# meteorologytoday/XLab-FFTBarotropic

Measured on AMD Instinct MI355X. Metric: RK4 steps/sec, 4096x4096 periodic grid, higher is better.
Workload: dtype f32; 1 GPU; 4096x4096 kuo2004 initial field, nu=6.5, L=600 km, dt=0.75 s, 4 RK stages/step, fused HIP path; parallelism=single

## Files before the change

### xlab-fftbarotropic_amd/csrc/fb_col_full.h

```cpp
#pragma once
#include "fb_kernels.h"

#define CF_THREADS 1024
#define CF_X1_CF 16384
#define CF_X2_STR 68
#define CF_X2_CF (16 * 16 * CF_X2_STR)
#define CF_GX_CF 2048
#define CF_LDS_CF (CF_X2_CF + 512 + CF_GX_CF)
#define CF_LDS_BYTES (CF_LDS_CF * 8)
#ifndef CF_KEEP1
#define CF_KEEP1 5
#endif
#ifndef CF_KEEP2
#define CF_KEEP2 5
#endif

struct FullArgs {
    const cf *Tin;
    const cf *Zbase;
    cf *Zcur, *Acc, *Zout;
    cf *W4;
    long fstride;
    int P;
    int ntiles;
    int ntiles_run;
    int nsub;
    int stage;
    float nu, dt;
    SpecCoef coef;
    const cf *tw256;
    const cf *tw4096;
    long sub_rows;
    float wscale;
};

FB_DEV void cf_xchg_waves(cf *lds, cf *v, int w, int lane)
{
#pragma unroll
    for (int r = 0; r < 16; ++r) lds_wr(&lds[(r * 16 + w) * 64 + lane], v[r]);
    lds_barrier();
#pragma unroll
    for (int r = 0; r < 16; ++r) v[r] = lds_rd(&lds[(w * 16 + r) * 64 + lane]);
    lds_barrier();
}

template <bool SYNC>
FB_DEV void cf_xchg_lanes(cf *lds, cf *v, int w, int l, int c)
{
    cf *reg = lds + w * (16 * CF_X2_STR);
#pragma unroll
    for (int r = 0; r < 16; ++r) lds_wr(&reg[r * CF_X2_STR + l * 4 + c], v[r]);
    __builtin_amdgcn_wave_barrier();
#pragma unroll
    for (int r = 0; r < 16; ++r) v[r] = lds_rd(&reg[l * CF_X2_STR + r * 4 + c]);
    if (SYNC) lds_barrier();
    else { asm volatile("s_waitcnt lgkmcnt(0)" ::: "memory"); __builtin_amdgcn_wave_barrier(); }
}

#define CF_FENCE() __builtin_amdgcn_sched_barrier(0)
FB_DEV cf cf_mul(cf a, cf b) { return cmul_split(a, b); }
FB_DEV cf cf_mulc(cf a, cf b) { return cmulc_split(a, b); }

template <int DIR> FB_DEV void cf_bfly16(cf *v)
{
    fft4<DIR>(v[0], v[4], v[8], v[12]);  CF_FENCE();
    fft4<DIR>(v[1], v[5], v[9], v[13]);  CF_FENCE();
// ... 191 lines not shown
#pragma unroll
        for (int k3 = 0; k3 < KEEP; ++k3) zkeep[k3] = cf_ld4(ZN + k3 * sstep, voff_s);
    }
#pragma unroll 1
    for (int f = 0; f < 4; ++f) {
        if (f > 0 || PRIME) {
            const unsigned vs = (unsigned)launder((int)voff_s);
#pragma unroll
            for (int k3 = 0; k3 < 16; ++k3) {
                const float4 z = k3 < KEEP ? zkeep[k3] : cf_ld4(ZN + k3 * sstep, vs);
                v[0][k3] = cf_make(z.x, z.y); v[1][k3] = cf_make(z.z, z.w);
            }
        }
        const bool psi = f >= 2, use_gx = (f == 0 || f == 3);
        const int lkx = launder(l);
#pragma unroll
        for (int k3 = 0; k3 < 16; ++k3) {
            cf za = v[0][k3], zb = v[1][k3];
            const float gx = gxt[16 * w + 256 * k3 + lkx];
            if (psi) {
                const double kx2 = (double)gx * (double)gx;
                const float lia = (nsub * (w + 256 * k3 + 16 * l) + k1 == 0 && ky0 == 0) ? 1.0f : (float)(-(kx2 + ky2_of(gya)));
                const float lib = (float)(-(kx2 + ky2_of(gyb)));
                za = pada ? cf_make(0.f, 0.f) : cf_make(za.x / lia, za.y / lia);
                zb = padb ? cf_make(0.f, 0.f) : cf_make(zb.x / lib, zb.y / lib);
            }
            const float ka = (use_gx ? gx : gya) * a.wscale, kb = (use_gx ? gx : gyb) * a.wscale;
            v[0][k3] = cf_make(-za.y * ka, za.x * ka);
            v[1][k3] = cf_make(-zb.y * kb, zb.x * kb);
            CF_FENCE();
        }
        cf_fft4096<+1, (KEEP > 0)>(lds, tabA, tabB, v, w, KEEP > 0 ? lkx : l, c, lane);
        char *dst = reinterpret_cast<char *>(a.W4) + (size_t)f * a.fstride * sizeof(cf) + ubase_m;
        const unsigned vm = (unsigned)launder((int)voff_m);
#pragma unroll
        for (int i = 0; i < 16; ++i)
            cf_st4_w4(dst + i * rstep, vm, make_float4(v[0][i].x, v[0][i].y, v[1][i].x, v[1][i].y));
    }
}

template <bool TO_FULL>
__global__ void __launch_bounds__(256) k_full_relayout(const cf *__restrict__ in, cf *__restrict__ out, int P, int N1, int N2, int ntiles, int nsub, int hy)
{
    const size_t total = (size_t)nsub * (ntiles + 1) * 16 * CF_THREADS * 2;
    for (size_t idx = (size_t)blockIdx.x * blockDim.x + threadIdx.x; idx < total; idx += (size_t)gridDim.x * blockDim.x) {
        const int col = (int)(idx & 1);
        const int tid = (int)((idx >> 1) & (CF_THREADS - 1));
        const int k3 = (int)((idx >> 11) & 15);
        const int st = (int)(idx >> 15);
        const int k1 = st / (ntiles + 1), tile = st - k1 * (ntiles + 1);
        const int w = tid >> 6, l = (tid >> 2) & 15, c = tid & 3;
        const int kx = nsub * (w + 16 * l + 256 * k3) + k1, ky = tile * 8 + 2 * c + col;
        const int cc = kx % N1, d = kx / N1;
        const size_t p3 = (size_t)(N2 * cc + d) * P + ky;
        if (ky >= hy) { if (TO_FULL) out[idx] = cf_make(0.f, 0.f); continue; }
        if (TO_FULL) out[idx] = in[p3]; else out[p3] = in[idx];
    }
}
```

### xlab-fftbarotropic_amd/csrc/fb_rowq.h

```cpp
#pragma once
#include "fb_rowh.h"

#define RQ_LAUNDER(t) (SLAB ? launder(t) : (t))
struct RowQ {
    static constexpr int M = 2048, N = 4096, T = 256;
    static constexpr int SLICE = Row8::SLICE;
    static constexpr int XBUF = 4 * SLICE;
    static constexpr int STG = M + 2;
    static constexpr int TW2 = 64;
    static constexpr size_t LDS_BYTES = (size_t)(XBUF + STG + TW2) * sizeof(cf);
};
struct RowQTw { cf w0[7], w1[3]; const cf *w2; };

FB_DEV void rq_xch_group_bwd(cf *v, cf *xbuf, int w, int l)
{
#pragma unroll
    for (int p = 0; p < 8; ++p) lds_wr(&xbuf[(p & 3) * RowQ::SLICE + ((p >> 2) * 4 + w) * 64 + l], v[p]);
    lds_barrier();
#pragma unroll
    for (int j = 0; j < 8; ++j) v[j] = lds_rd(&xbuf[w * RowQ::SLICE + j * 64 + l]);
}
FB_DEV void rq_xch_group_fwd(cf *v, cf *xbuf, int w, int l)
{
#pragma unroll
// ... 18 lines not shown
#pragma unroll
        for (int q = 1; q < 4; ++q) v[4 * h + q] = cmulc(v[4 * h + q], tw.w1[q - 1]);
    }
    r8_xch_wave<true>(v, slice, l_hi, l_lo);
    Bfly<8, +1>::run(v);
#pragma unroll
    for (int p = 1; p < 8; ++p) v[p] = cmulc(v[p], lds_rd(&tw.w2[p * 8 + l_lo]));
    r8_xch_wave<false>(v, slice, l_hi, l_lo);
    Bfly<8, +1>::run(v);
}

FB_DEV void rq_fwd(cf *v, cf *xbuf, const RowQTw &tw, int w, int l)
{
    const int l_hi = l >> 3, l_lo = l & 7;
    cf *slice = xbuf + w * RowQ::SLICE;
    Bfly<8, -1>::run(v);
    r8_xch_wave<false>(v, slice, l_hi, l_lo);
#pragma unroll
    for (int p = 1; p < 8; ++p) v[p] = cmul(v[p], lds_rd(&tw.w2[p * 8 + l_lo]));
    Bfly<8, -1>::run(v);
    r8_xch_wave<true>(v, slice, l_hi, l_lo);
#pragma unroll
    for (int h = 0; h < 2; ++h) {
#pragma unroll
        for (int q = 1; q < 4; ++q) v[4 * h + q] = cmul(v[4 * h + q], tw.w1[q - 1]);
        fft4<-1>(v[4 * h], v[4 * h + 1], v[4 * h + 2], v[4 * h + 3]);
    }
    rq_xch_group_fwd(v, xbuf, w, l);
#pragma unroll
    for (int p = 1; p < 8; ++p) v[p] = cmul(v[p], tw.w0[p - 1]);
    Bfly<8, -1>::run(v);
}

template <bool SLAB>
FB_DEV void rq_dma_issue(cf *stg, int t, const RowView &view, int field, int row)
{
    constexpr int M = RowQ::M;
    const int w = t >> 6, lane = t & 63;
#pragma unroll
    for (int c = 0; c < 4; ++c) {
        const int ch = w + c * 4, k = ch * 128 + lane * 2;
        __builtin_amdgcn_global_load_lds((const void __attribute__((address_space(1))) *)row_ptr<SLAB>(view, field, row, k), rh_to_lds(stg + ch * 128), 16, 0, 2);
    }
    rh_lds_ptr nyq = rh_to_lds(stg + M);
    const float *src = reinterpret_cast<const float *>(row_ptr<SLAB>(view, field, row, M)) + (t & 1);
    if (t < 2) __builtin_amdgcn_global_load_lds((const void __attribute__((address_space(1))) *)src, nyq, 4, 0, 0);
}

FB_DEV void rq_ext(cf *v, int t, const cf *stg, const cf *wk)
{
    constexpr int M = RowQ::M;
#pragma unroll
    for (int e = 0; e < 8; ++e) {
        const int k = t + 256 * e;
        cf a = lds_rd(&stg[k]), b = lds_rd(&stg[M - k]);
        if (e == 0 && t == 0) { a.y = 0.f; b.y = 0.f; }
        const cf ev = cadd_conj(a, b);
        cf d = cmul(csub_conj(a, b), wk[e == 4 ? 0 : e]);
        if (e == 4) d = mul_w16<4, +1>(d);
        v[e] = cadd_ib(ev, d);
    }
}

FB_DEV int rq_phys(int t, int e)
{
    const int w = t >> 6, l = t & 63, l_hi = l >> 3, l_lo = l & 7;
    return (w + 4 * (l_hi >> 2)) + 8 * (l_hi & 3) + 32 * l_lo + 256 * e;
}

__global__ void __launch_bounds__(256) k_rowq_permute_src(const float *__restrict__ in, float *__restrict__ out, int nrows)
{
    constexpr int M = RowQ::M;
    const size_t total = (size_t)nrows * M;
    for (size_t idx = (size_t)blockIdx.x * blockDim.x + threadIdx.x; idx < total; idx += (size_t)gridDim.x * blockDim.x) {
        const int x = (int)(idx / M), r = (int)(idx - (size_t)x * M);
        const int t = r & 255, e = r >> 8;
        reinterpret_cast<float2 *>(out)[idx] = reinterpret_cast<const float2 *>(in)[(size_t)x * M + rq_phys(t, e)];
    }
}

template <bool SLAB, bool PRE = false>
__global__ void __launch_bounds__(256, 4) k_rowq(RowArgs a, const float4 *__restrict__ tab )
{
    constexpr int M = RowQ::M;
    extern __shared__ __attribute__((aligned(16))) unsigned char smem_raw[];
    cf *xbuf = reinterpret_cast<cf *>(smem_raw);
    cf *stg = xbuf + RowQ::XBUF;
    const int t = threadIdx.x, l = t & 63;
    const bool valid = (int)blockIdx.x < a.nx;
    const int x = a.x0 + (valid ? (int)blockIdx.x : 0);
    rq_dma_issue<SLAB>(stg, t, a.M, 0, x);
    RowQTw tw;
    cf wkn[8];
    cf *tw2 = stg + RowQ::STG;
    {
        float4 q[9];
#pragma unroll
        for (int j = 0; j < 9; ++j) q[j] = tab[j * 256 + t];
        tw.w0[0] = cf_make(q[0].x, q[0].y); tw.w0[1] = cf_make(q[0].z, q[0].w); tw.w0[2] = cf_make(q[1].x, q[1].y); tw.w0[3] = cf_make(q[1].z, q[1].w);
        tw.w0[4] = cf_make(q[2].x, q[2].y); tw.w0[5] = cf_make(q[2].z, q[2].w); tw.w0[6] = cf_make(q[3].x, q[3].y);
        tw.w1[0] = cf_make(q[3].z, q[3].w); tw.w1[1] = cf_make(q[4].x, q[4].y); tw.w1[2] = cf_make(q[4].z, q[4].w);
        wkn[0] = cf_make(q[5].x, -q[5].y);
        if (t < 64) tw2[t] = cf_make(q[5].z, q[5].w);
        wkn[1] = cf_make(q[6].x, -q[6].y); wkn[2] = cf_make(q[6].z, -q[6].w); wkn[3] = cf_make(q[7].x, -q[7].y);
        wkn[5] = cf_make(q[7].z, -q[7].w); wkn[6] = cf_make(q[8].x, -q[8].y); wkn[7] = cf_make(q[8].z, -q[8].w);
        wkn[4] = wkn[0];
    }
    tw.w2 = tw2;
#pragma unroll
    for (int p = 0; p < 7; ++p) asm volatile("" :: "v"(tw.w0[p]));
    asm volatile("" :: "v"(tw.w1[0]), "v"(tw.w1[1]), "v"(tw.w1[2]), "v"(wkn[0]), "v"(wkn[7]));
    RH_WAIT_ROW();
    __syncthreads();

    for (int once = 0; once < 1; ++once) {
        cf v[8], p[8];
        auto c2r_phase = [&](bool wait, int next_field, int next_row) {
            const int tp = RQ_LAUNDER(t);
            if (wait) RH_WAIT_ROW();
            lds_barrier();
            rq_ext(v, tp, stg, wkn);
            lds_barrier();
            if (next_row >= 0) rq_dma_issue<SLAB>(stg, tp, a.M, next_field, next_row);
            rq_bwd(v, xbuf, tw, tp >> 6, tp & 63);
        };
        c2r_phase(false, 2, x);
#pragma unroll
        for (int e = 0; e < 8; ++e) p[e] = PRE ? v[e] : cf_make(v[e].x * a.scale, v[e].y * a.scale);
        c2r_phase(true, 1, x);
#pragma unroll
        for (int e = 0; e < 8; ++e) p[e] = PRE ? cf_make(v[e].x * p[e].x, v[e].y * p[e].y) : cf_make((v[e].x * a.scale) * p[e].x, (v[e].y * a.scale) * p[e].y);
        c2r_phase(true, 3, x);
        {
            cf zy[8];
#pragma unroll
            for (int e = 0; e < 8; ++e) zy[e] = PRE ? v[e] : cf_make(v[e].x * a.scale, v[e].y * a.scale);
            c2r_phase(true, 0, -1);
#pragma unroll
            for (int e = 0; e < 8; ++e)
                v[e] = PRE ? cf_make(p[e].x - v[e].x * zy[e].x, p[e].y - v[e].y * zy[e].y)
                           : cf_make(p[e].x - (v[e].x * a.scale) * zy[e].x, p[e].y - (v[e].y * a.scale) * zy[e].y);
        }
        const int tt = RQ_LAUNDER(t);
        if (a.src && a.src_nz[x]) {
            const float2 *sp = reinterpret_cast<const float2 *>(a.src) + (size_t)x * M + tt;
#pragma unroll
            for (int e = 0; e < 8; ++e) { const float2 q = sp[e * 256]; v[e].x += q.x; v[e].y += q.y; }
        }
        rq_fwd(v, xbuf, tw, tt >> 6, tt & 63);
        RH_WAIT_ROW();
        lds_barrier();
#pragma unroll
        for (int e = 4; e < 8; ++e) lds_wr(&xbuf[tt + 256 * (e - 4)], v[e]);
        lds_barrier();
        if (valid) {
#pragma unroll
// ... 24 lines not shown
```

### xlab-fftbarotropic_amd/csrc/fftbaro.hip

```cpp
#include <hip/hip_runtime.h>
#include <algorithm>
#include <cmath>
#include <cstdio>
#include <cstdlib>
#include <cstring>
#include <mutex>
#include <set>
#include <string>
#include <type_traits>
#include <utility>
#include <vector>

#include "../../include/fftbaro.h"
#include "fb_kernels.h"
#include "fb_keff.h"
#include "fb_azim.h"
#include "fb_census.h"
#include "fb_spectra.h"
#include "fb_tracer.h"
#include "fb_particles.h"
#include "fb_tangent.h"
#include "fb_clv.h"
#include "fb_adjoint.h"
#include "fb_obs.h"
// ... 54 lines not shown
    RK_GENERIC,
    RK_ROWQ,
    RK_ROW8,
    RK_ROWH_8192,
    RK_ROWH_16384,
    RK_ROWH2,
};
enum XPass {
    XP_COLS = 0,
    XP_FULL1 = 1,
    XP_FULL2 = 2,
};

struct fb_ctx {
    int world, rank;
    int XL;
    int ngroups, nact; ColGroup grp[3];
    int KA, KF, katot;
    int nx, ny, hy, P;
    int N1, N2;
    int jmax;
    float lx, ly;
    hipStream_t stream;
    RowKernel row;
    float *d_gx; double *d_kx2; float *d_gy; double *d_ky2; double gws;
    cf *d_tw_n1, *d_tw_n2, *d_tw_big, *d_tw_row_bwd, *d_tw_row_fwd, *d_tw_256;
    cf *d_tw_row3;
    cf *d_tw_4096;
    cf *d_tw_2048;
    bool rowq_off, no_row8, no_rowh;
    bool full_pass_off, full_noskip;
    bool no_column_skip, no_prescale;
    bool full_keep_off;
    int pitch_extra;
    bool no_pitch_tune, pitch_tune, tune_verbose;
    bool nyq_frozen;
    cf *d_scratch;
    std::vector<float> h_gx, h_gy; std::vector<double> h_kx2, h_ky2;
    int max_wg;
    int dev;
};

static void split_nx(int nx, int &N1, int &N2)
{
    if (nx % 3 == 0) { N1 = 24; N2 = nx / 24; return; }
    switch (nx) {
    case 64: N1 = 8; N2 = 8; break;
    case 128: N1 = 16; N2 = 8; break;
    case 256: N1 = 16; N2 = 16; break;
    case 512: N1 = 32; N2 = 16; break;
    case 1024: N1 = 32; N2 = 32; break;
    case 2048: N1 = 64; N2 = 32; break;
    case 4096: N1 = 64; N2 = 64; break;
    case 8192: N1 = 128; N2 = 64; break;
    default: N1 = 128; N2 = 128; break;
    }
}

static std::vector<cf> make_root_table(int n)
{
    std::vector<cf> t(n);
    for (int j = 0; j < n; ++j) {
        double a = -2.0 * M_PI * (double)j / (double)n;
        t[j].x = (float)cos(a); t[j].y = (float)sin(a);
    }
    return t;
// ... 45 lines not shown
    for (int s = 0; s < RowPlan<N>::S; ++s) r.push_back(RowTw<N, false>::radix(s));
    if (fwd) r = std::vector<int>(r.rbegin(), r.rend());
    return r;
}

static std::vector<int> plan_radices_rt(int n, bool fwd)
{
    switch (n) {
    case 64: return plan_radices<64>(fwd);
    case 128: return plan_radices<128>(fwd);
    case 256: return plan_radices<256>(fwd);
    case 512: return plan_radices<512>(fwd);
    case 1024: return plan_radices<1024>(fwd);
    case 2048: return plan_radices<2048>(fwd);
    case 4096: return plan_radices<4096>(fwd);
    case 8192: return plan_radices<8192>(fwd);
    default: return plan_radices<16384>(fwd);
    }
}

template <typename T> static int upload(T **dptr, const std::vector<T> &h)
{
    HIPCHK(hipMalloc((void **)dptr, h.size() * sizeof(T)));
    HIPCHK(hipMemcpy(*dptr, h.data(), h.size() * sizeof(T), hipMemcpyHostToDevice));
    return FB_OK;
}

static int autotune_pitch(fb_ctx *c);

static void read_switches(fb_ctx *c)
{
    auto set = [](const char *name) { return getenv(name) != nullptr; };
    const char *rowq = getenv("FB_ROWQ"), *full = getenv("FB_FULL_PASS"), *extra = getenv("FB_PITCH_EXTRA"), *keep = getenv("FB_FULL_KEEP");
    c->rowq_off = rowq && rowq[0] == '0';
    c->no_row8 = set("FB_NO_ROW8");
    c->no_rowh = set("FB_NO_ROWH");
    c->full_pass_off = full && full[0] == '0';
    c->full_noskip = set("FB_FULL_NOSKIP");
    c->no_column_skip = set("FB_NO_COLUMN_SKIP");
    c->no_prescale = set("FB_NO_PRESCALE");
    c->full_keep_off = keep && keep[0] == '0';
    c->pitch_extra = extra ? atoi(extra) : 0;
    c->no_pitch_tune = extra || set("FB_NO_PITCH_TUNE");
    c->pitch_tune = set("FB_PITCH_TUNE");
    c->tune_verbose = set("FB_TUNE_VERBOSE");
}

extern "C" int fb_create(fb_ctx **out, int nx, int ny, float lx, float ly) { return fb_create_slab(out, nx, ny, lx, ly, 0, 1); }

static int round16(int v) { return (v + 15) / 16 * 16; }

struct SlabLayout {
    double gws;
    int jmax;
    int XL, KA, KF;
    int nact, cols[2];
    int nfg, nch;
    bool two_streams;
};

static SlabLayout slab_layout(int nx, int ny, int world)
{
    SlabLayout L;
    const int dxw = (int)ceil(((double)(float)nx) / 3.0), dyw = (int)ceil(((double)(float)ny) / 3.0);
    L.gws = (double)(float)((double)dxw * dxw + (double)dyw * dyw);
    const int hy = ny / 2 + 1;
    L.jmax = 0;
    while (L.jmax < hy && (double)L.jmax * (double)L.jmax < L.gws) ++L.jmax;
    L.XL = nx / world;
    L.KA = round16((L.jmax + world - 1) / world);
    const int nf = hy - world * L.KA;
    L.KF = nf > 0 ? round16((nf + world - 1) / world) : 0;
    L.nact = 1;
    if (world > 1 && L.KA >= 32) {
// ... 297 lines not shown

static int set_max_lds(const fb_ctx *c, const void *fn, size_t bytes)
{
    static std::mutex mu; static std::set<std::pair<const void *, int>> done;
    std::lock_guard<std::mutex> lk(mu);
    if (done.count({fn, c->dev})) return FB_OK;
    HIPCHK(hipFuncSetAttribute(fn, hipFuncAttributeMaxDynamicSharedMemorySize, (int)bytes));
    done.insert({fn, c->dev});
    return FB_OK;
}

template <typename K, typename... A> static int launch_lds(const fb_ctx *c, K kern, int grid, int block, size_t lds, const A &...args)
{
    if (int rc = set_max_lds(c, (const void *)kern, lds)) return rc;
    return launch(c, kern, dim3(grid), dim3(block), lds, args...);
}

template <int N, int MODE> static int launch_row_t(fb_ctx *c, const RowArgs &a)
{
    using C = RowCfg<N>;
    constexpr int ppw = (C::PAIR2 && MODE == ROW_FUSED) ? C::G / 2 : C::G;
    const int grid = std::min((a.nx / 2 + ppw - 1) / ppw, c->max_wg / 2);
    return launch_lds(c, c->world > 1 ? k_row<N, MODE, true> : k_row<N, MODE, false>, grid, C::THREADS, C::LDS_BYTES, a);
}

template <int M, int MODE> static int launch_row3_t(fb_ctx *c, const RowArgs &a)
{
    using C = Row3Cfg<M>;
    constexpr int ppw = (C::TWO && MODE == ROW_FUSED) ? 1 : C::GP;
    const int grid = std::min((a.nx / 2 + ppw - 1) / ppw, c->max_wg);
    return launch_lds(c, c->world > 1 ? k_row3<M, MODE, true> : k_row3<M, MODE, false>, grid, C::THREADS, C::LDS_BYTES, a, (const cf *)c->d_tw_row3);
}

template <int MODE> static int launch_row(fb_ctx *c, RowArgs a, RowKernel k = RK_GENERIC)
{
    if (a.nx <= 0) return FB_OK;
    const bool slab = c->world > 1;
    if (MODE == ROW_FUSED) switch (k) {
    case RK_ROWQ:
        return launch_lds(c, slab ? k_rowq<true, false> : a.prescaled ? k_rowq<false, true> : k_rowq<false, false>, a.nx, 256, RowQ::LDS_BYTES,
                          a, (const float4 *)c->d_tw_2048);
    case RK_ROW8:
        if (a.nx < 2) break;
        return launch_lds(c, slab ? k_row8<true> : k_row8<false>, std::min(a.nx / 2, c->max_wg / 4), 512, Row8::LDS_BYTES, a, (const cf *)c->d_tw_row3);
    case RK_ROWH_8192:
        return launch_lds(c, slab ? k_rowh<1, true> : k_rowh<1, false>, std::min(a.nx, c->max_wg / 4), 512, RowH<1>::LDS_BYTES,
                          a, (const cf *)c->d_tw_4096, (const cf *)c->d_tw_row3);
    case RK_ROWH_16384:
        return launch_lds(c, slab ? k_rowh<2, true> : k_rowh<2, false>, std::min(a.nx, c->max_wg / 8), 512, RowH<2>::LDS_BYTES,
                          a, (const cf *)c->d_tw_4096, (const cf *)c->d_tw_row3);
    case RK_ROWH2:
        a.nx = 4096; a.sub_rows = 4096; a.tw_x = c->d_tw_big;
        return launch_lds(c, k_rowh2, std::min(a.nx, c->max_wg / 8), 1024, RowH2::LDS_BYTES, a, (const cf *)c->d_tw_4096, (const cf *)c->d_tw_row3);
    case RK_GENERIC: break;
    }
    switch (c->ny) {
    case 192: return launch_row3_t<64, MODE>(c, a);
    case 384: return launch_row3_t<128, MODE>(c, a);
    case 768: return launch_row3_t<256, MODE>(c, a);
    case 1536: return launch_row3_t<512, MODE>(c, a);
    case 3072: return launch_row3_t<1024, MODE>(c, a);
    case 64: return launch_row_t<64, MODE>(c, a);
    case 128: return launch_row_t<128, MODE>(c, a);
    case 256: return launch_row_t<256, MODE>(c, a);
    case 512: return launch_row_t<512, MODE>(c, a);
    case 1024: return launch_row_t<1024, MODE>(c, a);
    case 2048: return launch_row_t<2048, MODE>(c, a);
    case 4096: return launch_row_t<4096, MODE>(c, a);
    case 8192: return launch_row_t<8192, MODE>(c, a);
    case 16384: return launch_row_t<16384, MODE>(c, a);
    }
    return fail(FB_EUNSUPPORTED, "row pass: unsupported ny");
}

// ... 66 lines not shown
    const dim3 g(a.split ? (unsigned)(ntiles < c->max_wg ? ntiles : c->max_wg) : (unsigned)col_grid(c, ntiles)), b(256);
    switch (c->N2) {
    case 8: hipLaunchKernelGGL((k_col_mid<8>), g, b, 0, c->stream, a); break;
    case 16: hipLaunchKernelGGL((k_col_mid<16>), g, b, 0, c->stream, a); break;
    case 32: hipLaunchKernelGGL((k_col_mid<32>), g, b, 0, c->stream, a); break;
    case 64: hipLaunchKernelGGL((k_col_mid<64>), g, b, 0, c->stream, a); break;
    case 128: hipLaunchKernelGGL((k_col_mid<128>), g, b, 0, c->stream, a); break;
    default: return fail(FB_EUNSUPPORTED, "col mid: N2");
    }
    HIPCHK(hipGetLastError());
    return FB_OK;
}

static size_t priv_elems(const fb_ctx *c) { return grp_elems(c, c->grp[0]); }

static void finish_groups(fb_ctx *c)
{
    for (int g = 0; g < c->ngroups; ++g) {
        ColGroup &G = c->grp[g];
        const int act = (c->jmax - G.ky0 + 15) / 16;
        G.nct_active = act < 0 ? 0 : (act > G.ncols / 16 ? G.ncols / 16 : act);
        if (c->no_column_skip) G.nct_active = G.ncols / 16;
    }
}

static XPass choose_xpass(const fb_ctx *c)
{
    if (c->world != 1 || !c->nyq_frozen || ((c->ny / 2) % 8) != 0 || c->full_pass_off) return XP_COLS;
    if (c->nx == 4096) return XP_FULL1;
    if (c->nx == 8192 && c->row == RK_ROWH_8192) return XP_FULL2;
    return XP_COLS;
}

static int launch_full(const fb_ctx *c, const FullArgs &a)
{
    using K = void (*)(FullArgs);
#define CF_ROW(N, KP) {k_col_full<0, N, KP>, k_col_full<1, N, KP>, k_col_full<2, N, KP>, k_col_full<3, N, KP>, k_col_full<4, N, KP>}
    static const K ks[2][2][5] = {{CF_ROW(1, 0), CF_ROW(2, 0)},
                                  {CF_ROW(1, CF_KEEP1), CF_ROW(2, CF_KEEP2)}};
#undef CF_ROW
    return launch_lds(c, ks[c->full_keep_off ? 0 : 1][a.nsub - 1][a.stage], a.nsub * (a.stage == 4 ? a.ntiles + 1 : a.ntiles), CF_THREADS, CF_LDS_BYTES, a);
}

static int autotune_pitch(fb_ctx *c)
{
    finish_groups(c);
    if (c->world != 1 || c->no_pitch_tune) return FB_OK;
    if ((size_t)c->nx * c->P * sizeof(cf) < ((size_t)32 << 20)) return FB_OK;
    const XPass xp = choose_xpass(c);
    const int P0 = c->P, NC = xp != XP_COLS ? 7 : 4;
    constexpr int PITCH_HEADROOM = 96, RULE_EXTRA = 32;
    static_assert(RULE_EXTRA <= PITCH_HEADROOM && 16 * (7 - 1) <= PITCH_HEADROOM, "pitch candidates must fit the table head-room of create_impl");
    if ((int)c->h_gy.size() < P0 + PITCH_HEADROOM) return fail(FB_EINVAL, "autotune_pitch: coefficient tables shorter than the pitch candidates");
    hipDeviceProp_t prop;
    int dev = 0;
    const bool is_gfx950 = hipGetDevice(&dev) == hipSuccess && hipGetDeviceProperties(&prop, dev) == hipSuccess && strncmp(prop.gcnArchName, "gfx950", 6) == 0;
    if (xp != XP_COLS && is_gfx950 && !c->pitch_tune) {
        c->P = c->KA = c->katot = c->grp[0].ncols = P0 + RULE_EXTRA;
        finish_groups(c);
        return FB_OK;
    }
    const size_t maxe = (size_t)c->nx * (P0 + 16 * (NC - 1));
    const int nbuf = xp != XP_COLS ? 9 : 1;
    cf *buf = nullptr;
    if (hipMalloc((void **)&buf, maxe * nbuf * sizeof(cf)) != hipSuccess) { hipGetLastError(); return FB_OK; }
    hipMemsetAsync(buf, 0, maxe * nbuf * sizeof(cf), c->stream);
    hipEvent_t e0, e1;
    hipEventCreate(&e0); hipEventCreate(&e1);
    auto probe = [&](int P) -> int {
        ColGroup G = c->grp[0]; G.ncols = P;
        if (xp == XP_COLS) return launch_col_strided<+1>(c, G, buf, 1, 0);
        FullArgs a; memset(&a, 0, sizeof(a));
        a.Tin = buf; a.W4 = buf + maxe; a.Zbase = buf + 5 * maxe; a.Zcur = buf + 6 * maxe; a.Acc = buf + 7 * maxe; a.Zout = buf + 8 * maxe;
        a.fstride = (long)c->nx * P; a.P = P; a.ntiles = (c->ny / 2) / 8;
        a.ntiles_run = a.ntiles; a.nsub = xp; a.stage = 1; a.nu = 0.f; a.dt = 0.f; a.coef = make_coef(c); a.tw256 = c->d_tw_256;
        a.tw4096 = xp == XP_FULL1 ? c->d_tw_big : c->d_tw_4096; a.sub_rows = 4096;
        return launch_full(c, a);
    };
    const bool verbose = c->tune_verbose;
    hipEventRecord(e0, c->stream);
    for (int it = 0; it < 400; ++it) {
        if (probe(P0) != FB_OK) break;
        if ((it & 7) == 7) {
            hipEventRecord(e1, c->stream); hipEventSynchronize(e1);
            float ms = 0.f;
            if (hipEventElapsedTime(&ms, e0, e1) != hipSuccess || ms > 30.f) break;
        }
    }
    float tbest[8]; for (int k = 0; k < NC; ++k) tbest[k] = 1e30f;
    for (int rep = 0; rep < 6; ++rep)
        for (int k = 0; k < NC; ++k) {
            hipEventRecord(e0, c->stream);
            const int rc = probe(P0 + 16 * k);
            hipEventRecord(e1, c->stream);
            hipEventSynchronize(e1);
            float ms = 0.f;
            if (rc == FB_OK && hipEventElapsedTime(&ms, e0, e1) == hipSuccess && ms < tbest[k]) tbest[k] = ms;
        }
    float best = 1e30f; int bestP = P0;
    for (int k = 0; k < NC; ++k) {
        if (verbose) fprintf(stderr, "fftbaro: pitch probe P=%d %.4f ms\n", P0 + 16 * k, tbest[k]);
        if (tbest[k] < best * 0.99f) { best = tbest[k]; bestP = P0 + 16 * k; }
    }
    if (verbose) fprintf(stderr, "fftbaro: pitch %d -> %d\n", P0, bestP);
    c->P = c->KA = c->katot = c->grp[0].ncols = bestP;
    finish_groups(c);
    hipEventDestroy(e0); hipEventDestroy(e1);
    hipFree(buf);
    hipGetLastError();
// ... 85 lines not shown
{
    if (!c || !d_in || !d_out) return fail(FB_EINVAL, "fb_r2c: NULL");
    NEED_SINGLE(c);
    int rc;
    if ((rc = ensure_scratch(c))) return rc;
    HIPCHK(hipMemsetAsync(c->d_scratch, 0, priv_elems(c) * sizeof(cf), c->stream));
    if ((rc = r2c_private(c, d_in, c->d_scratch))) return rc;
    return relayout(c, c->d_scratch, (cf *)d_out, false);
}

extern "C" int fb_c2r(fb_ctx *c, const float *d_in, float *d_out, int normalize)
{
    if (!c || !d_in || !d_out) return fail(FB_EINVAL, "fb_c2r: NULL");
    NEED_SINGLE(c);
    int rc;
    if ((rc = ensure_scratch(c))) return rc;
    if ((rc = relayout(c, (const cf *)d_in, c->d_scratch, true))) return rc;
    const float scale = normalize ? 1.0f / (float)((size_t)c->nx * c->ny) : 1.0f;
    return c2r_private(c, c->d_scratch, d_out, scale);
}

struct GroupBufs { cf *ZA, *ZB, *ACC, *w4_send, *w4_recv, *t_send, *t_recv; };

struct Beside { cf *c0[3], *c1[3], *acc[3]; };
struct BesideSet { static constexpr int MAX = 32; Beside v[MAX]; int n; };
static_assert(FB_TANGENTS_MAX == BesideSet::MAX && FB_ADJOINTS_MAX == BesideSet::MAX, "BesideSet holds either public bound, and the refusals' text names it");

struct fb_model {
    fb_ctx *c;
    float nu, dt;
    GroupBufs gb[3];
    bool phase_flow;
    XPass xpass;
    bool prescale;
    bool use_graph, warmed;
    hipGraphExec_t graph_exec;
    const float *graph_src; hipStream_t graph_stream;
    float *src;
    int *src_nz;
    cf *rec_work[3], *rec_send[3];
    float *keff_fields;
    void *keff_red; size_t keff_red_cap;
    float *azim_fields;
    void *azim_red; size_t azim_red_cap;
    int *cs_label, *cs_ids;
    int2 *cs_part;
    float *pres_ref;
    unsigned char rec_work_nf[3], rec_send_nf[3];
    void *spec_red;
    int primed;
    Beside tr;
    float kappa;
    bool tracer;
    double *pt; int pt_n;
    float *pt_uv;
    double *pd;
    long long steps, pd_steps0;
    BesideSet tg;
    cf *tg_j[3];
    double *tg_red;
    float *rp_real;
    cf *tt[3]; int tt_depth, tt_fill;
    cf *ad_tape; int ad_depth, ad_fill;
    int ad_top;
    bool ad_on, ck_swept, ck_replay;
    int ck_every, ck_max, ck_n, ck_done, ck_left;
// ... 8 lines not shown
    double *pt_tape; int pt_depth, pt_fill;
    double *pa;
    unsigned long long *pa_acc;
    bool fr_on;
    ForcingArgs fr;
    int fr_nring;
    cf *fr_work;
    double *fr_part;
    unsigned long long *fr_dev;
};

#include "fb_transport.h"
struct fb_slab {
    fb_ctx *c;
    fb_model *m;
    fb_transport tp;
    bool connected, owns_streams;
    hipStream_t comp, comm;
    hipEvent_t ev_f[4], ev_r[8], ev_w4, ev_t, ev_tg[2], ev_rows_done, ev_fwd_done, ev_misc[2];
    int nfg, nch;
    int ncg;
    int step_ops;
};
#include "fb_entry.h"

static int model_create_impl(fb_model **out, fb_ctx *c, float nu, float dt, bool phase_flow)
{
    if (!out || !c) return fail(FB_EINVAL, "fb_model_create: NULL");
    *out = nullptr;
    fb_model *m = new fb_model();
    memset(m, 0, sizeof(*m));
    m->c = c; m->nu = nu; m->dt = dt; m->phase_flow = phase_flow;
    m->xpass = phase_flow ? XP_COLS : choose_xpass(c);
    m->prescale = m->xpass != XP_COLS && c->world == 1 && c->row == RK_ROWQ && !c->no_prescale;
    int rc = FB_OK;
    auto alloc0 = [&](cf **p, size_t elems) {
        if (rc || elems == 0) return;
        if (hipMalloc((void **)p, elems * sizeof(cf)) != hipSuccess) { rc = fail(FB_ENOMEM, "model allocation failed"); return; }
        if (hipMemsetAsync(*p, 0, elems * sizeof(cf), c->stream) != hipSuccess) rc = fail(FB_EHIP, "hipMemsetAsync failed");
    };
    for (int g = 0; g < c->ngroups; ++g) {
        const size_t n = grp_elems(c, c->grp[g]);
        GroupBufs &B = m->gb[g];
        alloc0(&B.ZA, n);
        if (g < c->nact) { alloc0(&B.ZB, n); alloc0(&B.ACC, n); }
        alloc0(&B.w4_send, 4 * n); alloc0(&B.t_send, n);
        if (c->world > 1) { alloc0(&B.w4_recv, 4 * n); alloc0(&B.t_recv, n); }
        else { B.w4_recv = B.w4_send; B.t_recv = B.t_send; }
    }
    if (rc) { fb_model_destroy(m); return rc; }
    *out = m;
    return FB_OK;
}

extern "C" int fb_model_create(fb_model **out, fb_ctx *c, float nu, float dt)
{
    if (c && c->world != 1) return fail(FB_EINVAL, "fb_model_create on a slab context: use fb_slab_create");
    return model_create_impl(out, c, nu, dt, false);
}

static int beside_stage(fb_model *m, fb_slab *s, int stage);
static void beside_step_done(fb_model *m);
static int forcing_stage(fb_model *m, fb_slab *s);
static size_t forcing_bytes(const fb_model *m);
static void beside_free_all(fb_model *m);
static size_t adjoint_bytes(const fb_model *m);
// ... 91 lines not shown
    const size_t half = (size_t)c->XL * c->ny / 2;
    switch (c->row) {
    case RK_ROWQ: return launch_n(c, k_rowq_permute_src, half, d_src, m->src, c->XL);
    case RK_ROWH_8192: return launch_n(c, k_rowh_permute_src<1>, half, d_src, m->src, c->XL);
    case RK_ROWH_16384: return launch_n(c, k_rowh_permute_src<2>, half, d_src, m->src, c->XL);
    default: HIPCHK(hipMemcpyAsync(m->src, d_src, n, hipMemcpyDeviceToDevice, c->stream)); return FB_OK;
    }
}
extern "C" int fb_model_set_source(fb_model *m, const float *d_src) { return set_source(on_model("fb_model_set_source", m), d_src); }
extern "C" int fb_slab_set_source_local(fb_slab *s, const float *d_rows) { return set_source(on_slab("fb_slab_set_source_local", s), d_rows); }

static MidArgs mid_args(fb_model *m, int g, int stage)
{
    fb_ctx *c = m->c;
    const ColGroup &G = c->grp[g];
    const GroupBufs &B = m->gb[g];
    MidArgs a;
    a.Tin = B.t_recv; a.Zbase = B.ZA; a.Zcur = B.ZB; a.Acc = B.ACC; a.Zout = B.ZA; a.W4 = B.w4_send;
    a.ct0 = 0; a.nct = stage < 0 ? G.ncols / 16 : G.nct_active;
    a.fstride = w4_fstride(c, G); a.rm = rowmap_w4(c, G); a.P = G.ncols; a.N1 = c->N1; a.N2 = c->N2; a.ky0 = G.ky0; a.stage = stage;
    a.nu = m->nu; a.dt = m->dt; a.coef = make_coef(c); a.tw_n = c->d_tw_n2; a.tw_big = c->d_tw_big;
    return a;
}

static int launch_col_full(fb_model *m, int stage)
{
    fb_ctx *c = m->c;
    const GroupBufs &B = m->gb[0];
    FullArgs a;
    a.Tin = B.t_recv; a.Zbase = B.ZA; a.Zcur = B.ZB; a.Acc = B.ACC; a.Zout = B.ZA; a.W4 = B.w4_send;
    a.fstride = (long)priv_elems(c); a.P = c->P; a.ntiles = (c->ny / 2) / 8; a.stage = stage; a.nu = m->nu; a.dt = m->dt;
    a.nsub = m->xpass; a.sub_rows = 4096;
    a.wscale = m->prescale ? 1.0f / (float)((size_t)c->nx * c->ny) : 1.0f;
    a.ntiles_run = c->grp[0].nct_active * 2 < a.ntiles ? c->grp[0].nct_active * 2 : a.ntiles;
    if (c->full_noskip) a.ntiles_run = a.ntiles;
    if (stage == 4) a.ntiles_run = a.ntiles + 1;
    a.coef = make_coef(c); a.tw256 = c->d_tw_256; a.tw4096 = m->xpass == XP_FULL1 ? c->d_tw_big : c->d_tw_4096;
    return launch_full(c, a);
}

static int full_import_state(fb_model *m, cf *spec3)
{
    fb_ctx *c = m->c;
    const int ntiles = (c->ny / 2) / 8;
    int rc;
    if ((rc = launch(c, k_full_relayout<true>, dim3(c->max_wg), dim3(256), 0, (const cf *)spec3, m->gb[0].ZA, c->P, c->N1, c->N2, ntiles, (int)m->xpass, c->hy)) ||
        (rc = launch_col_full(m, 4)))
        return rc;
    m->primed = 2;
    return FB_OK;
}

static int full_export_state(fb_model *m, cf *dst)
{
    fb_ctx *c = m->c;
    HIPCHK(hipMemsetAsync(dst, 0, priv_elems(c) * sizeof(cf), c->stream));
    const int ntiles = (c->ny / 2) / 8;
    return launch(c, k_full_relayout<false>, dim3(c->max_wg), dim3(256), 0, (const cf *)m->gb[0].ZA, dst, c->P, c->N1, c->N2, ntiles, (int)m->xpass, c->hy);
}

static int export_state(fb_model *m, int g, cf *dst)
{
    return m->xpass != XP_COLS ? full_export_state(m, dst) : state_convert(m->c, m->c->grp[g], m->gb[g].ZA, dst, false);
}

static int model_prime(fb_model *m)
{
    fb_ctx *c = m->c;
    int rc;
    for (int g = 0; g < c->ngroups; ++g) {
        const ColGroup &G = c->grp[g];
        if ((rc = launch_col_mid(c, mid_args(m, g, -1)))) return rc;
        if ((rc = launch_col_strided<+1>(c, G, m->gb[g].w4_send, 4, w4_fstride(c, G), rowmap_w4(c, G), G.nct_active, G.ncols / 16 - G.nct_active))) return rc;
    }
    m->primed = 1;
    return FB_OK;
}
static int model_col_bwd_active(fb_model *m, int f0 = 0, int f1 = 4, int g = 0)
{
    fb_ctx *c = m->c;
    const ColGroup &G = c->grp[g];
    return launch_col_strided<+1>(c, G, m->gb[g].w4_send + (size_t)f0 * w4_fstride(c, G), f1 - f0, w4_fstride(c, G), rowmap_w4(c, G), 0, G.nct_active);
}
static int launch_fused_row(fb_model *m, int x0, int nrows)
{
    fb_ctx *c = m->c;
    RowArgs a = row_args_base(c);
    if (c->world == 1) { a.M = view_single(c, m->gb[0].w4_recv, (long)priv_elems(c)); a.T = view_single(c, m->gb[0].t_send, 0); }
    else {
        const cf *w4[3] = {m->gb[0].w4_recv, m->gb[1].w4_recv, m->gb[2].w4_recv}, *ts[3] = {m->gb[0].t_send, m->gb[1].t_send, m->gb[2].t_send};
        a.M = view_slab(c, w4, 4); a.T = view_slab(c, ts, 1); a.t_frozen = 0;
    }
    a.src = m->src; a.src_nz = m->src_nz; a.scale = 1.0f / (float)((size_t)c->nx * c->ny); a.x0 = x0; a.nx = nrows; a.prescaled = m->prescale ? 1 : 0;
    return launch_row<ROW_FUSED>(c, a, m->xpass == XP_FULL2 ? RK_ROWH2 : c->row);
}
static int model_col_fwd(fb_model *m, int stage, int g = 0)
{
    fb_ctx *c = m->c;
    int rc;
    if ((rc = launch_col_strided<-1>(c, c->grp[g], m->gb[g].t_recv, 1, 0, rowmap_natural(), 0, c->grp[g].nct_active))) return rc;
    m->primed = 1;
    return launch_col_mid(c, mid_args(m, g, stage));
}

struct StepProf {
    std::vector<hipEvent_t> ev0[4], ev1[4];
    hipStream_t stream;
    int begin(int cls) { hipEvent_t a, b; if (hipEventCreate(&a) != hipSuccess || hipEventCreate(&b) != hipSuccess) return 1;
                         ev0[cls].push_back(a); ev1[cls].push_back(b); return hipEventRecord(a, stream) != hipSuccess; }
    int end(int cls) { return hipEventRecord(ev1[cls].back(), stream) != hipSuccess; }
};
#define PROF_BEGIN(cls) do { if (prof && prof->begin(cls)) return fail(FB_EHIP, "event record failed"); } while (0)
#define PROF_END(cls) do { if (prof && prof->end(cls)) return fail(FB_EHIP, "event record failed"); } while (0)

static int step_refusals(const Call &k, int nsteps)
{
    if (nsteps < 0) return refuse(k, "bad argument: nsteps < 0");
    if (int rc = enter(k, NEED_TRANSPORT)) return rc;
    const fb_model *m = k.m;
    if (m->ck_every) {
        if (nsteps > 0 && m->ck_swept) return refuse(k, "the window has been swept: start a new one (fb_model_set_vort, fb_model_set_spectrum, fb_model_adjoint_checkpoint)");
        if (nsteps > m->ck_max - m->ck_done)
            return refuse(k, "the checkpointed window has room for " + std::to_string(m->ck_max - m->ck_done) + " more steps (fb_model_adjoint_checkpoint)");
    } else if (m->ad_on && nsteps > m->ad_depth - m->ad_fill)
        return refuse(k, "the adjoint's tape has room for " + std::to_string(m->ad_depth - m->ad_fill) + " more steps (fb_model_adjoint_record)");
    if (m->pt_depth && nsteps > m->pt_depth - m->pt_fill)
        return refuse(k, "the particle tape has room for " + std::to_string(m->pt_depth - m->pt_fill) + " more steps (fb_model_particle_tape)");
// ... 124 lines not shown
```

Before: 1236 steps/s.

## Interleave W4 rows in pairs between column-full and rowq kernels

Adds a row-pair interleaved layout for the W4 intermediate buffer. The column-full kernel writes adjacent rows in 8-element chunks that alternate between the two rows, and k_rowq reads with the matching addressing and a remapped block index, so neighbouring workgroups consume interleaved rows. The aim is better write coalescing and locality on the column pass's strided stores and on the row pass's loads. It is enabled by default on a single GPU with the FULL1 pass and rowq, and it adds pitch and row-count constraints plus a different cache-policy flag on the loads.

```diff
diff --git a/xlab-fftbarotropic_amd/csrc/fb_col_full.h b/xlab-fftbarotropic_amd/csrc/fb_col_full.h
--- a/xlab-fftbarotropic_amd/csrc/fb_col_full.h
+++ b/xlab-fftbarotropic_amd/csrc/fb_col_full.h
@@ -32,6 +32,7 @@
     const cf *tw4096;
     long sub_rows;
     float wscale;
+    int w4_pairs;
 };
 
 FB_DEV void cf_xchg_waves(cf *lds, cf *v, int w, int lane)
@@ -289,7 +290,12 @@
         }
         cf_fft4096<+1, (KEEP > 0)>(lds, tabA, tabB, v, w, KEEP > 0 ? lkx : l, c, lane);
         char *dst = reinterpret_cast<char *>(a.W4) + (size_t)f * a.fstride * sizeof(cf) + ubase_m;
-        const unsigned vm = (unsigned)launder((int)voff_m);
+        unsigned vm = (unsigned)launder((int)voff_m);
+        if (NSUB == 1) {
+            const int pr = a.w4_pairs;
+            dst += (size_t)(pr * tile) * 8 * sizeof(cf);
+            vm += (unsigned)((launder(l) & 1) * (pr * (8 - a.P) * (int)sizeof(cf)));
+        }
 #pragma unroll
         for (int i = 0; i < 16; ++i)
             cf_st4_w4(dst + i * rstep, vm, make_float4(v[0][i].x, v[0][i].y, v[1][i].x, v[1][i].y));
diff --git a/xlab-fftbarotropic_amd/csrc/fb_rowq.h b/xlab-fftbarotropic_amd/csrc/fb_rowq.h
--- a/xlab-fftbarotropic_amd/csrc/fb_rowq.h
+++ b/xlab-fftbarotropic_amd/csrc/fb_rowq.h
@@ -74,7 +74,14 @@
     Bfly<8, -1>::run(v);
 }
 
-template <bool SLAB>
+template <bool SLAB, bool PAIR>
+FB_DEV const cf *rq_src_ptr(const RowView &v, int field, int row, int k)
+{
+    if (!PAIR) return row_ptr<SLAB>(v, field, row, k);
+    return v.a + (size_t)field * v.fstrA + (size_t)(row >> 1) * (2 * v.ka) + (row & 1) * 8 + ((k >> 3) * 16 + (k & 7));
+}
+
+template <bool SLAB, bool PAIR = false>
 FB_DEV void rq_dma_issue(cf *stg, int t, const RowView &view, int field, int row)
 {
     constexpr int M = RowQ::M;
@@ -82,10 +89,10 @@
 #pragma unroll
     for (int c = 0; c < 4; ++c) {
         const int ch = w + c * 4, k = ch * 128 + lane * 2;
-        __builtin_amdgcn_global_load_lds((const void __attribute__((address_space(1))) *)row_ptr<SLAB>(view, field, row, k), rh_to_lds(stg + ch * 128), 16, 0, 2);
+        __builtin_amdgcn_global_load_lds((const void __attribute__((address_space(1))) *)rq_src_ptr<SLAB, PAIR>(view, field, row, k), rh_to_lds(stg + ch * 128), 16, 0, PAIR ? 0 : 2);
     }
     rh_lds_ptr nyq = rh_to_lds(stg + M);
-    const float *src = reinterpret_cast<const float *>(row_ptr<SLAB>(view, field, row, M)) + (t & 1);
+    const float *src = reinterpret_cast<const float *>(rq_src_ptr<SLAB, PAIR>(view, field, row, M)) + (t & 1);
     if (t < 2) __builtin_amdgcn_global_load_lds((const void __attribute__((address_space(1))) *)src, nyq, 4, 0, 0);
 }
 
@@ -121,7 +128,7 @@
     }
 }
 
-template <bool SLAB, bool PRE = false>
+template <bool SLAB, bool PRE = false, bool PAIR = false>
 __global__ void __launch_bounds__(256, 4) k_rowq(RowArgs a, const float4 *__restrict__ tab )
 {
     constexpr int M = RowQ::M;
@@ -130,8 +137,9 @@
     cf *stg = xbuf + RowQ::XBUF;
     const int t = threadIdx.x, l = t & 63;
     const bool valid = (int)blockIdx.x < a.nx;
-    const int x = a.x0 + (valid ? (int)blockIdx.x : 0);
-    rq_dma_issue<SLAB>(stg, t, a.M, 0, x);
+    const int bx = PAIR ? (int)((((blockIdx.x >> 4) * 8 + (blockIdx.x & 7)) * 2) + ((blockIdx.x >> 3) & 1)) : (int)blockIdx.x;
+    const int x = a.x0 + (valid ? bx : 0);
+    rq_dma_issue<SLAB, PAIR>(stg, t, a.M, 0, x);
     RowQTw tw;
     cf wkn[8];
     cf *tw2 = stg + RowQ::STG;
@@ -163,7 +171,7 @@
             lds_barrier();
             rq_ext(v, tp, stg, wkn);
             lds_barrier();
-            if (next_row >= 0) rq_dma_issue<SLAB>(stg, tp, a.M, next_field, next_row);
+            if (next_row >= 0) rq_dma_issue<SLAB, PAIR>(stg, tp, a.M, next_field, next_row);
             rq_bwd(v, xbuf, tw, tp >> 6, tp & 63);
         };
         c2r_phase(false, 2, x);
diff --git a/xlab-fftbarotropic_amd/csrc/fftbaro.hip b/xlab-fftbarotropic_amd/csrc/fftbaro.hip
--- a/xlab-fftbarotropic_amd/csrc/fftbaro.hip
+++ b/xlab-fftbarotropic_amd/csrc/fftbaro.hip
@@ -110,6 +110,7 @@
     bool full_pass_off, full_noskip;
     bool no_column_skip, no_prescale;
     bool full_keep_off;
+    bool w4_pairs_off;
     int pitch_extra;
     bool no_pitch_tune, pitch_tune, tune_verbose;
     bool nyq_frozen;
@@ -221,6 +222,7 @@
 {
     auto set = [](const char *name) { return getenv(name) != nullptr; };
     const char *rowq = getenv("FB_ROWQ"), *full = getenv("FB_FULL_PASS"), *extra = getenv("FB_PITCH_EXTRA"), *keep = getenv("FB_FULL_KEEP");
+    const char *pairs = getenv("FB_W4_PAIRS");
     c->rowq_off = rowq && rowq[0] == '0';
     c->no_row8 = set("FB_NO_ROW8");
     c->no_rowh = set("FB_NO_ROWH");
@@ -229,6 +231,7 @@
     c->no_column_skip = set("FB_NO_COLUMN_SKIP");
     c->no_prescale = set("FB_NO_PRESCALE");
     c->full_keep_off = keep && keep[0] == '0';
+    c->w4_pairs_off = pairs && pairs[0] == '0';
     c->pitch_extra = extra ? atoi(extra) : 0;
     c->no_pitch_tune = extra || set("FB_NO_PITCH_TUNE");
     c->pitch_tune = set("FB_PITCH_TUNE");
@@ -592,14 +595,17 @@
     return launch_lds(c, c->world > 1 ? k_row3<M, MODE, true> : k_row3<M, MODE, false>, grid, C::THREADS, C::LDS_BYTES, a, (const cf *)c->d_tw_row3);
 }
 
-template <int MODE> static int launch_row(fb_ctx *c, RowArgs a, RowKernel k = RK_GENERIC)
+template <int MODE> static int launch_row(fb_ctx *c, RowArgs a, RowKernel k = RK_GENERIC, bool w4_pairs = false)
 {
     if (a.nx <= 0) return FB_OK;
     const bool slab = c->world > 1;
+    if (w4_pairs && (MODE != ROW_FUSED || k != RK_ROWQ || slab || a.x0 != 0 || (a.nx & 15) || a.M.ka < RowQ::M + 8))
+        return fail(FB_EINVAL, "row pass: the row-pair layout is k_rowq's on one GPU, over whole groups of sixteen rows");
     if (MODE == ROW_FUSED) switch (k) {
     case RK_ROWQ:
-        return launch_lds(c, slab ? k_rowq<true, false> : a.prescaled ? k_rowq<false, true> : k_rowq<false, false>, a.nx, 256, RowQ::LDS_BYTES,
-                          a, (const float4 *)c->d_tw_2048);
+        return launch_lds(c, slab ? k_rowq<true, false> : w4_pairs ? (a.prescaled ? k_rowq<false, true, true> : k_rowq<false, false, true>)
+                                                                   : (a.prescaled ? k_rowq<false, true> : k_rowq<false, false>),
+                          a.nx, 256, RowQ::LDS_BYTES, a, (const float4 *)c->d_tw_2048);
     case RK_ROW8:
         if (a.nx < 2) break;
         return launch_lds(c, slab ? k_row8<true> : k_row8<false>, std::min(a.nx / 2, c->max_wg / 4), 512, Row8::LDS_BYTES, a, (const cf *)c->d_tw_row3);
@@ -732,6 +738,11 @@
     return XP_COLS;
 }
 
+static bool w4_pairs_for(const fb_ctx *c, XPass xp)
+{
+    return c->world == 1 && xp == XP_FULL1 && c->row == RK_ROWQ && !c->w4_pairs_off;
+}
+
 static int launch_full(const fb_ctx *c, const FullArgs &a)
 {
     using K = void (*)(FullArgs);
@@ -775,6 +786,7 @@
         a.fstride = (long)c->nx * P; a.P = P; a.ntiles = (c->ny / 2) / 8;
         a.ntiles_run = a.ntiles; a.nsub = xp; a.stage = 1; a.nu = 0.f; a.dt = 0.f; a.coef = make_coef(c); a.tw256 = c->d_tw_256;
         a.tw4096 = xp == XP_FULL1 ? c->d_tw_big : c->d_tw_4096; a.sub_rows = 4096;
+        a.w4_pairs = w4_pairs_for(c, xp) ? 1 : 0;
         return launch_full(c, a);
     };
     const bool verbose = c->tune_verbose;
@@ -926,6 +938,7 @@
     GroupBufs gb[3];
     bool phase_flow;
     XPass xpass;
+    bool w4_pairs;
     bool prescale;
     bool use_graph, warmed;
     hipGraphExec_t graph_exec;
@@ -1000,6 +1013,7 @@
     memset(m, 0, sizeof(*m));
     m->c = c; m->nu = nu; m->dt = dt; m->phase_flow = phase_flow;
     m->xpass = phase_flow ? XP_COLS : choose_xpass(c);
+    m->w4_pairs = w4_pairs_for(c, m->xpass);
     m->prescale = m->xpass != XP_COLS && c->world == 1 && c->row == RK_ROWQ && !c->no_prescale;
     int rc = FB_OK;
     auto alloc0 = [&](cf **p, size_t elems) {
@@ -1157,10 +1171,12 @@
     a.fstride = (long)priv_elems(c); a.P = c->P; a.ntiles = (c->ny / 2) / 8; a.stage = stage; a.nu = m->nu; a.dt = m->dt;
     a.nsub = m->xpass; a.sub_rows = 4096;
     a.wscale = m->prescale ? 1.0f / (float)((size_t)c->nx * c->ny) : 1.0f;
+    a.w4_pairs = m->w4_pairs ? 1 : 0;
     a.ntiles_run = c->grp[0].nct_active * 2 < a.ntiles ? c->grp[0].nct_active * 2 : a.ntiles;
     if (c->full_noskip) a.ntiles_run = a.ntiles;
     if (stage == 4) a.ntiles_run = a.ntiles + 1;
     a.coef = make_coef(c); a.tw256 = c->d_tw_256; a.tw4096 = m->xpass == XP_FULL1 ? c->d_tw_big : c->d_tw_4096;
+    if (a.w4_pairs && 16 * (a.ntiles + 1) > 2 * a.P) return fail(FB_EINVAL, "k_col_full: the pitch is too short for the row-pair layout");
     return launch_full(c, a);
 }
 
@@ -1217,7 +1233,7 @@
         a.M = view_slab(c, w4, 4); a.T = view_slab(c, ts, 1); a.t_frozen = 0;
     }
     a.src = m->src; a.src_nz = m->src_nz; a.scale = 1.0f / (float)((size_t)c->nx * c->ny); a.x0 = x0; a.nx = nrows; a.prescaled = m->prescale ? 1 : 0;
-    return launch_row<ROW_FUSED>(c, a, m->xpass == XP_FULL2 ? RK_ROWH2 : c->row);
+    return launch_row<ROW_FUSED>(c, a, m->xpass == XP_FULL2 ? RK_ROWH2 : c->row, m->w4_pairs);
 }
 static int model_col_fwd(fb_model *m, int stage, int g = 0)
 {
```

New measurement: 1215 steps/s. 1.7% lower.
